# Sthiber/COSC_4397_Pathtracing_Raytracing_Project

Measured on AMD Instinct MI355X. Metric: Msamples/s, cornell.txt 1920x1080 depth 8 (+PSNR vs 5000spp ref), higher is better.
Workload: dtype f32

## Files before the change

### cosc_4397_pathtracing_raytracing_project_amd/capi.py

```python
from __future__ import annotations

import ctypes as C
import os
from typing import Optional, Sequence, Tuple

import numpy as np

_PKG = os.path.dirname(os.path.abspath(__file__))
LIB_PATH = os.environ.get("PT_AMD_LIB") or os.path.join(_PKG, "libpt_amd.so")
PT_MAX_DEPTH = 64
ARITH = {"exact": 0, "fma": 1, "fast": 2}
ARITH_NAMES = {v: k for k, v in ARITH.items()}
FEATURE_PLANES = 3
NOISE_PLANES = 2
NOISE_PIXELS_PER_PARTIAL = 1024
CONVERGENCE_WAVES = 16
CONVERGENCE_CAPACITY = 65536
FLT_MAX = float(np.finfo(np.float32).max)


class PtGeom(C.Structure):
    _fields_ = [("type", C.c_int32), ("materialid", C.c_int32), ("transform", C.c_float * 16),
                ("inverseTransform", C.c_float * 16), ("invTranspose", C.c_float * 16)]

# ... 13 lines not shown
class PtBVHNode(C.Structure):
    _fields_ = [("bmin", C.c_float * 3), ("bmax", C.c_float * 3), ("left", C.c_int32), ("right", C.c_int32),
                ("geomIndex", C.c_int32)]


class PtGridInfo(C.Structure):
    _fields_ = [("res", C.c_int32 * 3), ("origin", C.c_float * 3), ("cell_size", C.c_float * 3), ("pad", C.c_float),
                ("num_cells", C.c_int32), ("num_records", C.c_int32), ("num_leaves", C.c_int32)]


class PtGridRecord(C.Structure):
    _fields_ = [("bmin", C.c_float * 3), ("bmax", C.c_float * 3), ("leaf", C.c_int32), ("neighbours", C.c_int32)]


class PtSceneDesc(C.Structure):
    _fields_ = [("geoms", C.POINTER(PtGeom)), ("num_geoms", C.c_int32), ("materials", C.POINTER(PtMaterial)),
                ("num_materials", C.c_int32), ("camera", PtCamera), ("trace_depth", C.c_int32)]


class PtOptions(C.Structure):
    _fields_ = [("device", C.c_int32), ("pixel_begin", C.c_int32), ("pixel_count", C.c_int32),
                ("iters_per_batch", C.c_int32), ("num_queues", C.c_int32), ("blocks_per_cu", C.c_int32),
                ("time_kernels", C.c_int32), ("legacy_traversal", C.c_int32), ("debug_flags", C.c_int32), ("unfused_primary", C.c_int32), ("unfused_bounces", C.c_int32), ("stripe_pixels", C.c_int32), ("stripe_stride", C.c_int32),
                ("arith", C.c_int32), ("aa_jitter", C.c_int32), ("convergence", C.c_int32),
                ("lds_table_kb", C.c_int32), ("primary_pieces", C.c_int32), ("paths_pieces", C.c_int32), ("paths_min_piece", C.c_int32)]


class PtStats(C.Structure):
    _fields_ = [("samples", C.c_int64), ("live_rays", C.c_int64 * PT_MAX_DEPTH), ("intersect_launches", C.c_int64),
                ("intersect_ms", C.c_double), ("render_ms", C.c_double), ("num_cus", C.c_int32),
                ("grid_blocks", C.c_int32), ("num_queues", C.c_int32), ("iters_per_batch", C.c_int32),
                ("device_bytes", C.c_int64), ("primary_fused", C.c_int32), ("bounces_fused", C.c_int32),
                ("arith", C.c_int32), ("grid_cells", C.c_int32), ("tight_leaves", C.c_int32), ("paths_waves", C.c_int32), ("record_form", C.c_int32),
                ("gather_form", C.c_int32)]


class PtDenoiseOptions(C.Structure):
    _fields_ = [("levels", C.c_int32), ("sigma_color", C.c_float), ("sigma_normal", C.c_float), ("sigma_position", C.c_float),
                ("keep_albedo", C.c_int32)]


class PtSetupTimes(C.Structure):
    _fields_ = [("tables_ms", C.c_double), ("upload_ms", C.c_double), ("buffers_ms", C.c_double), ("probe_ms", C.c_double),
                ("set_camera_ms", C.c_double), ("set_camera_calls", C.c_int32)]


class PtError(RuntimeError):
    pass


_lib: Optional[C.CDLL] = None
_fp = C.POINTER(C.c_float)
_ip = C.POINTER(C.c_int32)


def lib() -> C.CDLL:
    global _lib
    if _lib is not None:
        return _lib
    if not os.path.exists(LIB_PATH):
        raise PtError(f"{LIB_PATH} not found: run `python -c 'import __graft_entry__ as g; g.build()'` "
                      "(hipcc --offload-arch=gfx950).  There is no CPU fallback.")
    L = C.CDLL(LIB_PATH)
    L.pt_last_error.restype = C.c_char_p
    L.pt_scene_load.argtypes = [C.c_char_p, C.c_int, C.c_int, C.POINTER(C.c_void_p)]
    L.pt_scene_free.argtypes = [C.c_void_p]
    L.pt_scene_free.restype = None
# ... 948 lines not shown
```

### cosc_4397_pathtracing_raytracing_project_amd/csrc/pt_api.cpp

```cpp
#include <chrono>
#include <cmath>
#include <cstdarg>
#include <cstdio>
#include <cstring>
#include <string>

#include "pt_adaptive.h"
#include "pt_context.h"
#include "pt_lds.h"
#include "pt_scene.h"
#include "pt_sched.h"

namespace {

std::string g_err;
constexpr int kDebugFlags = 16 | 32 | 64 | 128 | 256 | 512 | ptk::kRetireEveryIteration | 2048 | ptk::kWholeRecords | ptk::kNoFirstBounce | ptk::kRecordsByVisit | ptk::kTileGather;
static_assert(sizeof(PtOptions) == 80, "capi.PtOptions mirrors this layout");
static_assert(PT_CONVERGENCE_WAVES == ptk::kConvWaves, "pt_amd.h documents the size of the convergence metric's partial sums");
}
int pt_fail(const char* fmt, ...) {
  char buf[1024];
  va_list ap;
  va_start(ap, fmt);
  vsnprintf(buf, sizeof(buf), fmt, ap);
  va_end(ap);
  g_err = buf;
  return -1;
}

namespace ptc {
static PtContext* g_default = nullptr;
PtContext* default_context() { return g_default; }

int get_events(Ctx& g, EventPair* ev) {
  if (!g.free_events.empty()) {
    *ev = g.free_events.back();
    g.free_events.pop_back();
    return 0;
  }
  HIP_OK(hipEventCreate(&ev->a));
  HIP_OK(hipEventCreate(&ev->b));
  return 0;
}
static int resolve_events(Ctx& g) {
  auto drain = [&](std::vector<EventPair>& pending, double& total_ms) -> int {
    for (auto& e : pending) {
      float ms = 0;
      HIP_OK(hipEventElapsedTime(&ms, e.a, e.b));
      total_ms += ms;
// ... 50 lines not shown
ptk::BatchInfo tile_batch(const Ctx& g, int iter_first, int K) {
  ptk::BatchInfo b{};
  b.iter_first = iter_first;
  b.K = K;
  b.N = g.N;
  b.pixel_begin = g.pixel_begin;
  b.trace_depth = g.depth;
  b.aa_jitter = g.aa_jitter ? 1 : 0;
  b.stripe = g.stripe;
  b.gap = g.stripe ? g.stripe_stride - g.stripe : 0;
  b.inv_stripe = g.stripe ? 1.0f / (float)g.stripe : 0.0f;
  return b;
}

int run_batch(Ctx& g, int iter_first, int kb) {
  ptk::BatchInfo b = tile_batch(g, iter_first, kb);
  b.slot_shift = g.slot_shift;
  b.flat = g.fuse_bounces ? 0 : 1;
  b.primary_share = primary_share_of(g);
  b.primary_pieces = g.primary_pieces ? g.primary_pieces
                     : ptk::primary_shares(b) ? ptk::auto_shared_pieces(kb, g.qs.nq, g.ret.wq0) : ptk::auto_primary_pieces(kb, g.qs.nq, g.ret.wq0);
  b.paths_pieces = g.paths_pieces;
  const ptk::SceneTables sc = tables(g);
  b.retire_once = ptk::retires_once(b, g.debug_flags) ? 1 : 0;
  b.split_records = ptk::record_form(b, g.debug_flags, ptk::search_form(sc), sc.num_mats);
  if (b.split_records == ptk::kFirstBounce) b.primary_pieces = 1;
  g.record_form = b.split_records;
  b.fixed_slots = ptk::fixed_slots(b, g.debug_flags, ptk::search_form(sc), sc.num_mats, g.ret.seg_cap) ? 1 : 0;
  b.list = g.list;
  if (b.list) b.stripe = 1, b.gap = 0, b.inv_stripe = 1.0f;
  const ptk::KernelApi& k = *g.k;
  auto cnt_row = [&](int d) { return g.d_cnt + ptk::cnt_index(g.qs, d, 0); };
  int d0 = 0;
  if (g.fuse_primary) {
    k.primary(g.stream, g.grid_primary, sc, g.dcam, b, queues_for(g, g.grid_primary), cnt_row(0), cnt_row(1), g.buf[1],
              g.ret);
    d0 = 1;
  } else {
    k.generate(g.stream, g.grid_gen, g.dcam, b, queues_for(g, g.grid_gen), g.buf[0], cnt_row(0));
  }
  int src = d0 & 1;
  const bool all_depths = g.grid_paths > 0;
  EventPair ev{};
  auto timed_from = [&]() -> int {
    if (!g.time_kernels) return 0;
    if (get_events(g, &ev)) return -1;
    HIP_OK(hipEventRecord(ev.a, g.stream));
    return 0;
  };
  auto timed_to = [&]() -> int {
    if (!g.time_kernels) return 0;
    HIP_OK(hipEventRecord(ev.b, g.stream));
    g.pending_isect.push_back(ev);
    return 0;
  };
  if (all_depths) {
    if (timed_from()) return -1;
    k.paths(g.stream, g.grid_paths, sc, b, queues_for(g, g.grid_paths), g.d_cnt, g.buf[1], g.ret);
    if (timed_to()) return -1;
  }
  for (int d = d0; d < g.depth && !all_depths; ++d) {
    const int32_t* cin = cnt_row(d);
    int32_t* cout = cnt_row(d + 1);
    if (timed_from()) return -1;
    k.intersect(g.stream, g.grid_isect, sc, queues_for(g, g.grid_isect), cin, g.buf[src], g.hits, g.legacy, d == 0);
    if (timed_to()) return -1;
    k.shade(g.stream, g.grid_shade, sc, b, d, queues_for(g, g.grid_shade), cin, cout, g.buf[src], g.hits, g.buf[src ^ 1], g.ret);
    src ^= 1;
  }
  ptk::ConvInfo cv{g.d_ref, g.d_partial, -1, kb};
  if (g.conv_live) {
    if (g.conv_have_ref) cv.first_k = 0;
    else if (g.conv >= iter_first && g.conv < iter_first + kb) cv.capture_k = g.conv - iter_first, cv.first_k = cv.capture_k + 1, g.conv_have_ref = true;
    g.conv_last = std::max(g.conv_last, iter_first + kb - 1);
  }
  const bool conv_batch = cv.capture_k >= 0 || cv.first_k < kb;
  g.gather_form = ptk::gather_form(b.fixed_slots != 0, g.debug_flags, conv_batch);
  if (g.gather_form == ptk::kGatherStream) k.collect_stream(g.stream, b, g.qs, g.ret, g.d_image, g.d_cnt, g.depth, g.d_stats);
  else {
    k.count_stats(g.stream, g.qs, g.d_cnt, g.depth, g.d_stats);
    if (conv_batch) k.collect_conv(g.stream, b, g.qs, g.ret, g.d_image, cv, g.d_sse);
    else k.collect(g.stream, b, g.qs, g.ret, g.d_image);
  }
  HIP_OK(hipGetLastError());
  g.samples += (int64_t)kb * g.N;
  if (g.pending_isect.size() > 16384) {
    HIP_OK(hipStreamSynchronize(g.stream));
    if (resolve_events(g)) return -1;
  }
  return 0;
}

void plan_launch(Ctx& g) {
  if (!g.borrowed) g.lds_table_bytes = g.k->lds_table_limit(tables(g), g.lds_table_forced);
  const ptk::SceneTables t = tables(g);
  g.grid_gen = g.num_cus * std::min(g.cap_bpc, g.k->resident_blocks_per_cu(ptk::kGenerate, t));
  g.grid_isect = g.num_cus * std::min(g.cap_bpc, g.k->resident_blocks_per_cu(g.legacy ? ptk::kIntersectLegacy : ptk::kIntersect, t));
  g.grid_shade = g.num_cus * std::min(g.cap_bpc, g.k->resident_blocks_per_cu(ptk::kShade, t));
  g.grid_primary = g.num_cus * std::min(g.cap_bpc, g.k->resident_blocks_per_cu(shares_first_hit(g) ? ptk::kPrimaryShared : ptk::kPrimary, t));
  g.ret.wq0 = ptk::wave_slot(0, g.qs.Q, g.grid_primary * ptk::kWavesPerBlock).wq;
  g.grid_paths = (g.fuse_bounces && g.depth > 1) ? g.num_cus * std::min(g.cap_bpc, g.k->resident_blocks_per_cu(ptk::kPaths, t)) : 0;
  g.qs.paths_W = g.grid_paths * ptk::kWavesPerBlock;
}

static void free_grid(Ctx& g, const Ctx::DeviceGrid& d) {
  for (void* p : {(void*)d.d_start, (void*)d.d_items, d.d_items_b != d.d_items ? (void*)d.d_items_b : nullptr}) {
    if (!p) continue;
    (void)hipFree(p);
    g.allocs.erase(std::remove(g.allocs.begin(), g.allocs.end(), p), g.allocs.end());
  }
  g.device_bytes -= (int64_t)d.bytes;
}
static int choose_traversal(Ctx& g) {
  auto drop_unused_grids = [&](size_t keep) {
    for (size_t i = 0; i < g.grids.size(); ++i)
      if (i != keep) free_grid(g, g.grids[i]);
    g.grids = {g.grids[keep]};
    g.grid_pick = 0;
  };
  if (g.grids.empty()) return 0;
  if (!g.fuse_bounces || (g.debug_flags & (256 | 512))) {
    drop_unused_grids(0);
    return 0;
  }
  auto time_one = [&](float* ms) -> int {
    plan_launch(g);
    for (int rep = 0; rep < 2; ++rep) {
      EventPair ev{};
      if (get_events(g, &ev)) return -1;
      HIP_OK(hipEventRecord(ev.a, g.stream));
      if (run_batch(g, 1, std::min(g.K, 8))) return -1;
      HIP_OK(hipEventRecord(ev.b, g.stream));
      HIP_OK(hipStreamSynchronize(g.stream));
      HIP_OK(hipEventElapsedTime(ms, ev.a, ev.b));
      g.free_events.push_back(ev);
    }
    return 0;
  };
  g.grid_enabled = false;
  if (time_one(&g.probe_ms[0])) return -1;
  g.grid_enabled = true;
  size_t best = 0;
  for (size_t i = 0; i < g.grids.size(); ++i) {
    float ms = 0.f;
    g.grid_pick = i;
    if (time_one(&ms)) return -1;
    if (i == 0 || ms < 0.97f * g.probe_ms[1]) g.probe_ms[1] = ms, best = i;
  }
  drop_unused_grids(best);
  g.grid_enabled = g.probe_ms[1] < 0.95f * g.probe_ms[0];
  plan_launch(g);
  HIP_OK(hipMemsetAsync(g.d_image, 0, 3 * (size_t)g.N * sizeof(float), g.stream));
  HIP_OK(hipMemsetAsync(g.d_stats, 0, PT_MAX_DEPTH * sizeof(unsigned long long), g.stream));
  HIP_OK(hipStreamSynchronize(g.stream));
  g.samples = 0;
  return 0;
}

ptd::Queues single_queue(const Ctx& g, int n) {
  ptd::Queues qs{};
  qs.Q = 1;
  const ptk::QueuePlan p = ptk::queue_plan(n, 1, 1);
  qs.cap = p.cap;
  qs.W = g.grid * ptk::kWavesPerBlock;
  qs.cnt_stride = 16;
  qs.nq = p.nq;
  qs.inv_nq = 1.0f / (float)qs.nq;
  return qs;
}

void destroy(Ctx* c) {
  if (!c) return;
  destroy(c->worker);
  (void)hipSetDevice(c->device);
  if (c->stream) (void)hipStreamSynchronize(c->stream);
  for (void* p : c->allocs) (void)hipFree(p);
  auto kill = [](std::vector<EventPair>& v) {
    for (auto& e : v) {
      (void)hipEventDestroy(e.a);
      (void)hipEventDestroy(e.b);
    }
    v.clear();
  };
  kill(c->free_events);
  kill(c->pending_isect);
  kill(c->pending_render);
  if (c->stream && !c->borrowed) (void)hipStreamDestroy(c->stream);
  delete c;
// ... 121 lines not shown
static int upload_tables(Ctx& g, const pt::HostTables& t) {
  ptk::SceneTables& s = g.scene;
  s.num_nodes = (int)t.nodes.size(), s.num_geoms = (int)t.geoms.size(), s.num_mats = (int)t.mats.size(), s.num_top = (int)t.top.size();
  std::memcpy(s.root_min, t.root_min, 12);
  std::memcpy(s.root_max, t.root_max, 12);
  s.cull_margin = t.cull_margin;
  s.top_xor = t.top_xor;
  s.has_triangles = t.has_triangles ? 1 : 0;
  g.tight_leaves = t.tight_leaves;
  if (!(s.nodes = upload(g, t.nodes)) || !(s.geoms = upload(g, t.geoms)) || !(s.mats = upload(g, t.mats)) || !(s.top = upload(g, t.top))) return -1;
  s.nodes_b = s.nodes, s.top_b = s.top;
  if (!t.nodes_b.empty() && (!(s.nodes_b = upload(g, t.nodes_b)) || !(s.top_b = upload(g, t.top_b)))) return -1;
  for (const pt::Grid& gr : t.grids)
    if (upload_grid(g, gr)) return -1;
  return 0;
}

static __global__ void k_poison_records(ptd::Word4* rec, unsigned long long per_queue, unsigned long long total, int Q) {
  const float nan = __builtin_nanf("");
  for (unsigned long long i = (unsigned long long)blockIdx.x * blockDim.x + threadIdx.x; i < total; i += (unsigned long long)gridDim.x * blockDim.x)
    rec[i] = ptd::Word4{nan, nan, nan, __int_as_float(ptk::chunk_pixel((int)(i / per_queue), 0, Q))};
}

static int poison_records(Ctx& g) {
  const size_t regions = (size_t)g.qs.Q * g.ret.kmax, per_queue = (size_t)g.ret.kmax * g.ret.seg_cap;
  hipLaunchKernelGGL(k_poison_records, dim3((unsigned)std::min<size_t>((regions * g.ret.seg_cap + 255) / 256, 65536)), dim3(256), 0, g.stream, g.ret.rec,
                     (unsigned long long)per_queue, (unsigned long long)(regions * g.ret.seg_cap), g.qs.Q);
  HIP_OK(hipGetLastError());
  return 0;
}
static size_t sub_words_max(const Ctx& g) { return ptk::sub_stride(g.num_cus * 8 * ptk::kWavesPerBlock, g.qs.Q); }

static int rearm_batch_buffers(Ctx& g) {
  for (const ptd::PathBuf& pb : g.buf) HIP_OK(hipMemsetAsync(pb.r, 0xff, pathbuf_words(pb.stride) * sizeof(ptd::Word4), g.stream));
  const size_t regions = (size_t)g.qs.Q * g.ret.kmax;
  HIP_OK(hipMemsetAsync(g.ret.cnt, 0, regions * sizeof(*g.ret.cnt), g.stream));
  HIP_OK(hipMemsetAsync(g.ret.sub, 0, regions * sub_words_max(g) * sizeof(*g.ret.sub), g.stream));
  if (g.qs.deal) HIP_OK(hipMemsetAsync(g.qs.deal, 0, (size_t)ptk::deal_map(g.qs).words() * sizeof(int32_t), g.stream));
  return poison_records(g);
}

int alloc_batch_buffers(Ctx& g) {
  const int Q = g.qs.Q;
  if (alloc_pathbuf(g, &g.buf[0], g.stride) || alloc_pathbuf(g, &g.buf[1], g.stride)) return -1;
  for (const ptd::PathBuf& pb : g.buf) HIP_OK(hipMemset(pb.r, 0xff, pathbuf_words(pb.stride) * sizeof(ptd::Word4)));
  if (!g.fuse_bounces && alloc_hitbuf(g, &g.hits, g.stride)) return -1;
  {
    const size_t regions = (size_t)Q * g.ret.kmax;
    const size_t wq_max = sub_words_max(g);
    if (dalloc(g, &g.ret.rec, regions * g.ret.seg_cap)) return -1;
    if (ensure(g, g.ret.cnt, regions * sizeof(*g.ret.cnt), Zero::blocking) || ensure(g, g.ret.sub, regions * wq_max * sizeof(*g.ret.sub), Zero::blocking)) return -1;
    if (poison_records(g)) return -1;
  }
  const size_t image_bytes = 3 * (size_t)g.N * sizeof(float);
  const size_t cnt_words = ptk::cnt_index(g.qs, g.depth + 1, 0);
  if (ensure(g, g.d_image, image_bytes, Zero::blocking) || ensure(g, g.d_cnt, cnt_words * sizeof(int32_t), Zero::blocking) ||
      ensure(g, g.d_stats, PT_MAX_DEPTH * sizeof(*g.d_stats), Zero::blocking))
    return -1;
  if (!(g.debug_flags & 64) && ensure(g, g.qs.deal, (size_t)ptk::deal_map(g.qs).words() * sizeof(int32_t), Zero::blocking)) return -1;
  if (g.conv) {
    const size_t partials = (size_t)g.K * Q * ptk::kConvWaves;
    if (ensure(g, g.d_ref, image_bytes, Zero::blocking) || ensure(g, g.d_partial, partials * sizeof(double), Zero::blocking)) return -1;
    if (dalloc(g, &g.d_sse, (size_t)PT_CONVERGENCE_CAPACITY)) return -1;
    HIP_OK(hipMemset(g.d_sse, 0xff, (size_t)PT_CONVERGENCE_CAPACITY * sizeof(double)));
  }
  HIP_OK(hipDeviceSynchronize());
// ... 282 lines not shown
  (void)hipFree(d);
  if (e != hipSuccess) return pt_fail("pt_preview_rgba8: %s", hipGetErrorString(e));
  return 0;
}

int pt_ctx_get_stats(PtContext* c, PtStats* out) {
  if (need(c, "pt_get_stats")) return -1;
  if (!out) return pt_fail("pt_get_stats: null");
  if (pt_ctx_sync(c)) return -1;
  Ctx& g = *c;
  std::memset(out, 0, sizeof(*out));
  unsigned long long st[PT_MAX_DEPTH];
  HIP_OK(hipMemcpy(st, g.d_stats, sizeof(st), hipMemcpyDeviceToHost));
  for (int d = 0; d < PT_MAX_DEPTH; ++d) out->live_rays[d] = (int64_t)st[d];
  out->samples = g.samples;
  out->intersect_launches = g.isect_launches;
  out->intersect_ms = g.isect_ms;
  out->render_ms = g.render_ms;
  out->num_cus = g.num_cus;
  out->grid_blocks = g.grid_paths > 0 ? g.grid_paths : g.grid_isect;
  out->num_queues = g.qs.Q;
  out->iters_per_batch = g.K;
  out->device_bytes = g.device_bytes;
  out->primary_fused = g.fuse_primary ? 1 : 0;
  out->bounces_fused = g.fuse_bounces ? 1 : 0;
  out->arith = g.arith;
  if (tables(g).use_grid && g.fuse_bounces) {
    const int* res = g.grids[g.grid_pick].shape.res;
    out->grid_cells = res[0] * res[1] * res[2];
  }
  out->tight_leaves = g.tight_leaves;
  out->record_form = g.record_form;
  out->gather_form = g.gather_form;
  out->paths_waves = 0;
  if (g.qs.deal && g.grid_paths > 0) {
    const ptk::DealMap dm = ptk::deal_map(g.qs);
    std::vector<int32_t> first((size_t)dm.made_for() + 1);
    HIP_OK(hipMemcpy(first.data(), g.qs.deal + dm.first(0), first.size() * sizeof(int32_t), hipMemcpyDeviceToHost));
    if (first[dm.made_for()] == g.qs.paths_W) {
      int lo = first[1] - first[0], hi = lo;
      for (int q = 1; q < g.qs.Q; ++q) lo = std::min(lo, first[q + 1] - first[q]), hi = std::max(hi, first[q + 1] - first[q]);
      out->paths_waves = std::min(lo, 0xffff) << 16 | std::min(hi, 0xffff);
    }
  }
  return 0;
}

int pt_ctx_reset_stats(PtContext* c) {
  if (need(c, "pt_reset_stats")) return -1;
  if (pt_ctx_sync(c)) return -1;
  Ctx& g = *c;
  HIP_OK(hipMemsetAsync(g.d_stats, 0, PT_MAX_DEPTH * sizeof(unsigned long long), g.stream));
  HIP_OK(hipStreamSynchronize(g.stream));
  g.samples = 0;
  g.isect_ms = g.render_ms = 0;
  g.isect_launches = 0;
  return 0;
}

int pt_ctx_clear(PtContext* c) {
  if (need(c, "pt_clear")) return -1;
  if (pt_ctx_sync(c)) return -1;
  HIP_OK(hipMemsetAsync(c->d_image, 0, 3 * (size_t)c->N * sizeof(float), c->stream));
  if (c->d_feat) HIP_OK(hipMemsetAsync(c->d_feat, 0, (size_t)PT_FEATURE_PLANES * c->N * sizeof(float4), c->stream));
  if (c->d_noise) HIP_OK(hipMemsetAsync(c->d_noise, 0, pt_noise_state_bytes((size_t)c->N), c->stream));
  c->noise_groups = 0;
// ... 197 lines not shown
```

### cosc_4397_pathtracing_raytracing_project_amd/csrc/pt_context.h

```cpp
#pragma once
#include <hip/hip_runtime.h>

#include <algorithm>
#include <cstdint>
#include <vector>

#include "../../include/pt_amd.h"
#include "pt_device.h"
#include "pt_internal.h"
#include "pt_kernels.h"
#include "pt_tables.h"

#define HIP_OK(expr)                                                                                      \
  do {                                                                                                    \
    hipError_t e_ = (expr);                                                                               \
    if (e_ != hipSuccess) return pt_fail("%s failed: %s (%s:%d)", #expr, hipGetErrorString(e_), __FILE__, __LINE__); \
  } while (0)

struct EventPair {
  hipEvent_t a, b;
};

struct PtShared {
  int device = 0;
// ... 41 lines not shown
  int grid_gen = 0, grid_isect = 0, grid_shade = 0;
  ptd::Queues qs{};
  int64_t stride = 0;
  std::vector<void*> allocs;
  int64_t device_bytes = 0;
  float probe_ms[2] = {0.f, 0.f};
  int grid_primary = 0, grid_paths = 0;
  ptd::PathBuf buf[2]{};
  ptd::HitBuf hits{};
  ptd::RetireBuf ret{};
  float* d_image = nullptr;
  float4* d_feat = nullptr;
  int grid_features = 0;
  void* d_denoise = nullptr;
  void* d_noise = nullptr;
  int noise_groups = 0;
  int64_t noise_iters = 0;
  int64_t rendered = 0;
  int conv = 0;
  bool conv_live = false;
  bool conv_have_ref = false;
  int conv_last = 0;
  float* d_ref = nullptr;
  double* d_partial = nullptr;
  double* d_sse = nullptr;
  uint8_t* d_rgb8 = nullptr;
  int32_t* d_cnt = nullptr;
  unsigned long long* d_stats = nullptr;
  bool time_kernels = false;
  std::vector<EventPair> free_events, pending_isect, pending_render;
  double isect_ms = 0, render_ms = 0;
  int64_t isect_launches = 0;
  int64_t samples = 0;
  bool failed = false;
  int opt_iters_per_batch = 0, opt_num_queues = 0;
  bool borrowed = false;
  const int32_t* list = nullptr;
  PtContext* worker = nullptr;
  int capacity = 0;
  int32_t* d_list = nullptr;
  int32_t* d_list_frame = nullptr;
  void* d_acnt = nullptr;
  void* d_select = nullptr;
  float* d_resolved = nullptr;
  pt::CameraBase camera_base;
  pt::GridRequest grid_request;
  PtSetupTimes setup_times{};
  bool adaptive = false;
  int adaptive_rounds = 0;
  int64_t adaptive_last = 0;
};

struct PtCtxState {
  bool adaptive;
  int groups;
  int64_t iters;
  int64_t unfolded;
};
PtCtxState pt_ctx_state(const PtContext* c);
int pt_ctx_admit_state(const PtContext* c, const char* who, bool uniform);
int pt_ctx_adaptive_refusal(const PtContext* c, const char* who, int iter_first, int group_iters, float max_fraction, bool folds);
int pt_ctx_camera_refusal(const PtContext* c, const PtCamera* cam, const char* who);
int pt_ctx_enter_adaptive(PtContext* c);

namespace ptc {
using Ctx = PtContext;
// ... 72 lines not shown
```

### cosc_4397_pathtracing_raytracing_project_amd/csrc/pt_kernels.hip

```cpp
#include "pt_kernels.h"

#include <float.h>

#include <type_traits>

#include "pt_lds.h"
#include "pt_sched.h"
#include "pt_portable_math.h"

#ifndef PT_ARITH
#define PT_ARITH 0
#endif
#if PT_ARITH == 0
#define PT_NS arith_exact
#define PT_API_FN api_exact
#elif PT_ARITH == 1
#define PT_NS arith_fma
#define PT_API_FN api_fma
#elif PT_ARITH == 2
#define PT_NS arith_fast
#define PT_API_FN api_fast
#else
#error "PT_ARITH must be 0, 1 or 2"
#endif
// ... 1028 lines not shown
      if (dead) rt.rec[sub0 + nd + rank_in(deadm)] = ptd::Word4{s.c.x, s.c.y, s.c.z, __int_as_float(pl)};
      nl += (int)__popcll(live), nd += (int)__popcll(deadm);
    };
    if constexpr (RING) ws = carry_init<true, 2>(wbase), ws.qo_tab = cam_qo, ws.cam_o = o;
    if constexpr (SHARE && SPLIT == kFirstBounce) {
      const int sub_off = sub_offset(quo, rem, shared_rho(r, 0, wq)) * 64;
      int fnl = 0, fnd = 0;
      auto record_group = [&](unsigned long long best, const float* rec, const Group& g) {
        const bool valid = g.valid;
        const Hit h = resolve_hit(best, rec, valid, leaf_geom);
        const bool cdead = valid && (h.t < 0.0f || mats[h.mat].emittance > 0.0f), lives = valid && !cdead;
        const unsigned long long livem = ballot(lives), cdeadm = ballot(cdead);
        if (lives) path_store(out, qbase + sub_off + fnl + rank_in(livem), bounce_origin(h.n, h.p), h.n, g.d, PathTag{pack_first(g.pl, h.mat, b.slot_shift), g.phash, 0});
        if (cdead) {
          ShadeIO s;
          s.o = o;
          s.d = g.d;
          s.c = mk(1.0f, 1.0f, 1.0f);
          s.alive = false;
          shade_decide(mats, b.trace_depth, 0, iter_hash_of(ihash, sc, b, 0, 0) ^ g.phash, h.t, h.mat, s);
          rt.rec[sub_off + fnd + rank_in(cdeadm)] = ptd::Word4{s.c.x, s.c.y, s.c.z, __int_as_float(g.pl)};
        }
        fnl += (int)__popcll(livem), fnd += (int)__popcll(cdeadm);
      };
      pp.any = false;
      int it = 0;
      for (int jj = shared_rho(r, 0, wq); jj < sh.my_nq; jj += wq, ++it) trace(it, group_of(jj, 0), record_group);
      if constexpr (RING) {
        if (pp.any) {
          carry_drain_to<true, 2, kD0, true>(ws, pp.mark, lane, nodes, geoms);
          record_group(ws.best[pp.par * 64 + lane], ws.rec + pp.par * 6 * 64 + lane, pp.g);
        }
      }
      for (int k = lane; k < b.K; k += 64) rt.sub[k * rt.wq0 + shared_rho(r, k, wq)] = ((unsigned long long)(uint32_t)fnd << 32) | (uint32_t)fnl;
    } else if constexpr (SHARE) {
      const int cap = shared_run_cap(b.primary_share), sub_off = sub_offset(quo, rem, shared_rho(r, k0, wq)) * 64;
      const bool once = b.retire_once != 0;
      for (int run = 0, runs = shared_runs(k0, k1, cap); run < runs; ++run) {
        const Run sr = shared_run(k0, k1, cap, run);
        const int s0 = sr.k0, s1 = sr.k1;
        int vnl = 0, vnd = 0;
        auto shade_run = [&](unsigned long long best, const float* rec, const Group& g) {
          const bool valid = g.valid;
          const int pl = g.pl;
          const uint32_t phash = g.phash;
          const f3 d = g.d;
          const Hit h = resolve_hit(best, rec, valid, leaf_geom);
          const float ht = h.t;
          const int hmat = h.mat;
          const f3 hn = h.n, hp = h.p;
          if constexpr (SPLIT == kSplitRecords) {
            if (s0 == 0) {
              const bool lives = valid && !(ht < 0.0f || mats[hmat].emittance > 0.0f);
              const unsigned long long livem = ballot(lives);
              const f3 o1 = bounce_origin(hn, hp);
              if (lives) out.r[out.stride + qbase + sub_off + __builtin_amdgcn_readlane(vnl, 0) + rank_in(livem)] = ptd::Word4{o1.x, o1.y, o1.z, __int_as_float(hmat)};
            }
          }
          const bool cdead = once && valid && (ht < 0.0f || mats[hmat].emittance > 0.0f);
          const unsigned long long cdeadm = once ? ballot(cdead) : 0ull;
          if (once) {
            if (s0 == 0 && cdeadm) {
              ShadeIO s;
              s.o = o;
              s.d = d;
              s.c = mk(1.0f, 1.0f, 1.0f);
              s.alive = false;
// ... 237 lines not shown
    tword[e] = (uint32_t)leaf | ((uint32_t)gi << 8);
    lmat[leaf & 63] = sc.geoms[gi].material;
  }
  __syncthreads();
  const int wib = threadIdx.x >> 6;
  char* wbase = lds + L.waves + wib * L.wave_bytes;
  Lanes cy = lanes_init(wbase);
  GridRings gr = grid_rings_init<false>(wbase);
  Carry<false, 1>& cb = gr.cy;
  CellRing& cr = gr.cr;
  cb.lnodes = (const __attribute__((address_space(3))) v4f*)(lnodes ? lnodes : lds), cb.lds_nodes = lnodes != nullptr;
  constexpr bool SLOTS = MODE == 0;
  char* slots = wbase + WM::slots;
  int* died = reinterpret_cast<int*>(wbase + WM::died);
  [[maybe_unused]] int* fillc = reinterpret_cast<int*>(wbase + WM::fillc);
  const int ntop = sc.num_top;
  const int wave = __builtin_amdgcn_readfirstlane(blockIdx.x * kWavesPerBlock + wib);
  const int lane = lane_id();
  died[lane] = 0;
  const uint64_t t_begin = __builtin_amdgcn_s_memrealtime();
  const DealMap dm = deal_map(qs);
  const WaveSlot even = wave_slot(wave, qs.Q, qs.W);
  int q = even.q, r = even.r, wq = even.wq;
  if (qs.deal != nullptr && qs.deal[dm.made_for()] == qs.W) {
    int at_or_before = 0;
    for (int e0 = 0; e0 < qs.Q; e0 += 64) at_or_before += (int)__popcll(ballot(e0 + lane < qs.Q && qs.deal[dm.first(e0 + lane)] <= wave));
    q = at_or_before - 1;
    const int first = qs.deal[dm.first(q)];
    r = wave - first, wq = qs.deal[dm.first(q + 1)] - first;
  }
  const Retire rt = retire_of(ret, q);
  const int64_t qbase = (int64_t)q * qs.cap;
  const int wq0 = rt.wq0, ne = b.K * wq0;
  const int my_nq = queue_share(b, qs, q).my_nq, quo = my_nq / wq0, rem = my_nq % wq0;
  auto count_of = [&](int e) { return e < ne ? (int)(uint32_t)rt.sub[e] : 0; };
  int total = 0, csum = 0;
  const bool chunk_sums = ne <= 64 * 64;
  for (int e0 = 0; e0 < ne; e0 += 256) {
    int n4[4];
#pragma unroll
    for (int j = 0; j < 4; ++j) n4[j] = count_of(e0 + 64 * j + lane);
#pragma unroll
    for (int j = 0; j < 4; ++j) {
      int sum;
      (void)wave_prefix6(n4[j], sum);
      total += sum;
      if (lane == (e0 >> 6) + j) csum = sum;
    }
  }
  if (r == 0 && lane == 0) cnt[cnt_index(qs, 1, q)] = total;
  const PiecePlan pieces = piece_plan(total, wq, b.paths_pieces, qs.deal != nullptr, chunk_sums);
  [[maybe_unused]] int clist0 = 0;
  int ce = ne, cstart = total, ccnt = 0, clist = 0;
  int cord = 0;
  [[maybe_unused]] int cur_k = 0;
  [[maybe_unused]] uint32_t cur_h = 0u, next_h = 0u;
  [[maybe_unused]] int crec0 = 0;
  [[maybe_unused]] const int fbits = fixed_bits(rt.seg_cap);
  int win0 = -64;
  unsigned long long wsub = 0ull;
  auto window_to = [&](int e) {
    if (e < win0 || e >= win0 + 64) {
      win0 = e;
      wsub = (e + lane < ne) ? rt.sub[e + lane] : 0ull;
    }
  };
  auto sub_word = [&](int e) -> unsigned long long {
    const uint32_t lo32 = (uint32_t)__builtin_amdgcn_readlane((int)(uint32_t)wsub, e - win0);
    const uint32_t hi32 = (uint32_t)__builtin_amdgcn_readlane((int)(uint32_t)(wsub >> 32), e - win0);
    return ((unsigned long long)hi32 << 32) | lo32;
  };
  window_to(0);
  auto cursor_bases = [&](int first_rank) {
    const int ec = min(ce, ne - 1), ck = ec / wq0, crho = ec - ck * wq0;
    clist = ck * rt.seg_cap + sub_offset(quo, rem, crho) * 64;
    if constexpr (SPLIT != 0) clist0 = invariant_slot(clist, ck, rt.seg_cap);
    if constexpr (FIRST) cur_k = ck, cur_h = iter_hash(b.iter_first + ck, 0);
    window_to(ec);
    const int crec = clist + (int)(uint32_t)(sub_word(ec) >> 32);
    if constexpr (FIXED) crec0 = invariant_slot(crec, ck, rt.seg_cap);
    else if (lane == 0) fillc[cord & (kVisitRing - 1)] = crec + (first_rank - cstart);
  };
  auto seek = [&](int at_rank) {
// ... 395 lines not shown
```

### cosc_4397_pathtracing_raytracing_project_amd/csrc/pt_post.cpp

```cpp
#include <cmath>

#include "pt_adaptive.h"
#include "pt_context.h"
#include "pt_denoise.h"
#include "pt_noise.h"
#include "pt_sched.h"

using namespace ptc;

int64_t pt_ctx_unfolded_iterations(const PtContext* c) { return c ? c->rendered - c->noise_iters : 0; }

extern "C" {

int pt_ctx_render_features(PtContext* c, int iter_first, int iter_count) {
  if (need(c, "pt_render_features")) return -1;
  Ctx& g = *c;
  if (iter_first < 1 || iter_count < 0 || (int64_t)iter_first + iter_count - 1 > INT32_MAX)
    return pt_fail("pt_render_features: iterations %d, +%d: the first is >= 1, the count >= 0", iter_first, iter_count);
  if (admit(g, "pt_render_features", kNotFailed | kOnDevice)) return -1;
  const ptk::SceneTables sc = tables(g);
  static_assert(sizeof(float4) == 16, "a feature plane holds 16 bytes per pixel");
  if (ensure(g, g.d_feat, (size_t)PT_FEATURE_PLANES * g.N * sizeof(float4), Zero::on_stream)) return -1;
  if (iter_count == 0) return 0;
  const int groups = (g.N + 63) / 64;
// ... 141 lines not shown
void set_worker_live(Ctx& w, int m) {
  const ptk::QueuePlan plan = ptk::queue_plan(m, w.qs.Q, w.K);
  w.N = m;
  w.qs.nq = plan.nq;
  w.qs.inv_nq = 1.0f / (float)plan.nq;
  w.qs.cap = plan.cap;
  w.stride = (int64_t)w.qs.Q * plan.cap;
  w.ret.seg_cap = plan.seg_cap;
}

int ensure_worker(Ctx& g, int m) {
  if (g.worker && g.worker->capacity == m) return set_worker_live(*g.worker, m), 0;
  if (g.worker) g.device_bytes -= g.worker->device_bytes, destroy(g.worker), g.worker = nullptr;
  if (ensure(g, g.d_list, (size_t)g.N * sizeof(int32_t), Zero::blocking)) return -1;
  if (g.stripe && ensure(g, g.d_list_frame, (size_t)g.N * sizeof(int32_t), Zero::blocking)) return -1;
  Ctx* w = new Ctx();
  w->borrowed = true;
  static_cast<PtShared&>(*w) = g;
  PtOptions o{};
  o.pixel_begin = g.pixel_begin, o.pixel_count = m;
  o.iters_per_batch = g.opt_iters_per_batch, o.num_queues = g.opt_num_queues;
  if (plan_batches(*w, o)) return destroy(w), -1;
  plan_launch(*w);
  if (alloc_batch_buffers(*w)) return destroy(w), -1;
  w->list = g.stripe ? g.d_list_frame : g.d_list;
  w->capacity = m;
  g.worker = w;
  g.device_bytes += w->device_bytes;
  return 0;
}

int render_list(Ctx& g, int iter_first, int iter_count) {
  Ctx& w = *g.worker;
  HIP_OK(hipMemsetAsync(w.d_image, 0, 3 * (size_t)w.N * sizeof(float), g.stream));
  const int end = iter_first + iter_count;
  for (int it = iter_first; it < end; it += w.K)
    if (run_batch(w, it, std::min(w.K, end - it))) {
      g.failed = true;
      return -1;
    }
  return 0;
}

static int adaptive_refusal(const Ctx& g, const char* who, int iter_first, int group_iters, const float* fraction_or_null, bool folds = true,
                            bool rows = true) {
  const float fraction = fraction_or_null ? *fraction_or_null : 1.0f;
  if (admit(g, who, kNotFailed)) return -1;
  if (folds && (iter_first < 1 || group_iters < 1 || (int64_t)iter_first + group_iters - 1 > INT32_MAX))
    return pt_fail("%s: iterations %d, +%d: the first is >= 1, the group holds at least one", who, iter_first, group_iters);
  if (!folds && iter_first < 1) return pt_fail("%s: the first iteration %d is not >= 1", who, iter_first);
  if (!(fraction > 0.0f && fraction <= 1.0f)) return pt_fail("%s: fraction %g is not in (0, 1]", who, (double)fraction);
  if (g.conv) return pt_fail("%s: the renderer was created with PtOptions.convergence = %d; the convergence metric follows whole iterations", who, g.conv);
  if (rows && admit(g, who, kWholeRows)) return -1;
  if (g.adaptive || !folds) return 0;
  if (g.noise_groups < 2) return pt_fail("%s: %d group(s) folded; the selection needs the noise estimate of at least 2 (pt_noise_fold)", who, g.noise_groups);
  if (admit(g, who, kFoldedAll)) return -1;
  if (g.noise_iters > INT32_MAX / 2) return pt_fail("%s: %lld iterations folded: the per-pixel counts are int32", who, (long long)g.noise_iters);
  return 0;
}

static int enter_adaptive(Ctx& g) {
  if (g.adaptive) return 0;
  if (ensure(g, g.d_acnt, (size_t)g.N * sizeof(ptad::Cnt))) return -1;
  if (pt_adaptive_init_counts_launch(g.stream, g.N, g.d_acnt, (int)g.noise_iters, g.noise_groups)) return -1;
  g.adaptive = true;
  g.adaptive_rounds = 0;
// ... 210 lines not shown
```

### cosc_4397_pathtracing_raytracing_project_amd/csrc/pt_sched.h

```cpp
#pragma once
#include "pt_kernels.h"

#define PT_SCHED __host__ __device__ inline __attribute__((always_inline))

namespace ptk {

PT_SCHED int sched_min(int a, int b) { return a < b ? a : b; }
PT_SCHED int sched_max(int a, int b) { return a > b ? a : b; }

struct DealMap {
  int Q;
  PT_SCHED int first(int q) const { return q; }
  PT_SCHED int made_for() const { return Q; }
  PT_SCHED int time(int q) const { return Q + 1 + q; }
  PT_SCHED int strand_counter() const { return 2 * Q + 1; }
  PT_SCHED int piece_counter(int q) const { return 2 * Q + 2 + q; }
  PT_SCHED int rays(int q) const { return 3 * Q + 2 + q; }
  PT_SCHED int words() const { return 4 * Q + 2; }
};
PT_SCHED DealMap deal_map(const ptd::Queues& qs) { return DealMap{qs.Q}; }

PT_SCHED int dealt_first(int q, int W, int Q, unsigned long long work_before, unsigned long long work_total) {
  return q + (int)((unsigned long long)(W - Q) * work_before / work_total);
}
// ... 120 lines not shown
PT_SCHED bool splits_records(const BatchInfo& b, int debug_flags) {
  return splits_records(b.primary_share, b.aa_jitter != 0, b.flat != 0, b.trace_depth, debug_flags);
}
PT_SCHED int invariant_slot(int at, int k, int seg_cap) { return at - k * seg_cap; }
PT_SCHED uint32_t pack_kind(int sample_id, bool specular) { return (uint32_t)sample_id | (specular ? 0x80000000u : 0u); }
PT_SCHED int kind_sample_id(uint32_t word) { return (int)(word & 0x7fffffffu); }
PT_SCHED bool kind_specular(uint32_t word) { return (word >> 31) != 0u; }

constexpr int kNoFirstBounce = 8192;
constexpr int kSplitRecords = 1, kFirstBounce = 2;
constexpr int kVisitBits = 8;
PT_SCHED uint32_t pack_visit(int k, int visit) { return ((uint32_t)k << kVisitBits) | ((uint32_t)visit & ((1u << kVisitBits) - 1u)); }
PT_SCHED int visit_k(uint32_t word) { return (int)(word >> kVisitBits); }
PT_SCHED int visit_number(uint32_t word) { return (int)(word & ((1u << kVisitBits) - 1u)); }
PT_SCHED int visit_gap(int visits_now, int visit) { return (visits_now - visit) & ((1 << kVisitBits) - 1); }
PT_SCHED bool visit_k_fits(int K) { return K <= (1 << (31 - kVisitBits)); }
PT_SCHED int pack_first(int pl, int mat, int slot_shift) { return (mat << slot_shift) | pl; }
PT_SCHED int first_pixel(int word, int slot_shift) { return word & ((1 << slot_shift) - 1); }
PT_SCHED int first_material(int word, int slot_shift) { return (int)((uint32_t)word >> slot_shift); }
PT_SCHED bool first_material_fits(int num_mats, int slot_shift) { return num_mats <= (1 << (31 - slot_shift)); }
PT_SCHED bool first_bounces(int primary_share, bool aa_jitter, bool flat, int trace_depth, int debug_flags, int search_form, int num_mats,
                            int slot_shift, int K) {
  return splits_records(primary_share, aa_jitter, flat, trace_depth, debug_flags) &&
         retires_once(primary_share, aa_jitter, flat, trace_depth, debug_flags) && !(debug_flags & kNoFirstBounce) && search_form == 0 &&
         first_material_fits(num_mats, slot_shift) && visit_k_fits(K);
}
PT_SCHED bool first_bounces(const BatchInfo& b, int debug_flags, int search_form, int num_mats) {
  return first_bounces(b.primary_share, b.aa_jitter != 0, b.flat != 0, b.trace_depth, debug_flags, search_form, num_mats, b.slot_shift, b.K);
}
PT_SCHED int record_form(const BatchInfo& b, int debug_flags, int search_form, int num_mats) {
  return first_bounces(b, debug_flags, search_form, num_mats) ? kFirstBounce : splits_records(b, debug_flags) ? kSplitRecords : 0;
}

constexpr int kRecordsByVisit = 16384, kTileGather = 32768;
constexpr int kFixedSlots = 3;
PT_SCHED int fixed_slot(int k, int seg_cap, int quo, int rem, int rho, int retirees, int i) { return k * seg_cap + sub_offset(quo, rem, rho) * 64 + retirees + i; }
PT_SCHED int fixed_bits(int seg_cap) { return 32 - __builtin_clz((unsigned)(seg_cap - 1)); }
PT_SCHED uint32_t pack_fixed(int k, int in_region, int bits) { return ((uint32_t)k << bits) | (uint32_t)in_region; }
PT_SCHED int fixed_k(uint32_t word, int bits) { return (int)(word >> bits); }
PT_SCHED int fixed_slot_of(uint32_t word, int bits, int seg_cap) { return (int)(word >> bits) * seg_cap + (int)(word & ((1u << bits) - 1u)); }
PT_SCHED bool fixed_word_fits(int K, int seg_cap) { return K <= (1 << (31 - fixed_bits(seg_cap))); }
PT_SCHED bool fixed_slots(int primary_share, bool aa_jitter, bool flat, int trace_depth, int debug_flags, int search_form, int num_mats, int slot_shift,
                          int K, int seg_cap) {
  return first_bounces(primary_share, aa_jitter, flat, trace_depth, debug_flags, search_form, num_mats, slot_shift, K) && fixed_word_fits(K, seg_cap) &&
         !(debug_flags & kRecordsByVisit);
}
PT_SCHED bool fixed_slots(const BatchInfo& b, int debug_flags, int search_form, int num_mats, int seg_cap) {
  return fixed_slots(b.primary_share, b.aa_jitter != 0, b.flat != 0, b.trace_depth, debug_flags, search_form, num_mats, b.slot_shift, b.K, seg_cap);
}
constexpr int kGatherTile = 0, kGatherTileFixed = 1, kGatherStream = 2;
PT_SCHED int gather_form(bool fixed, int debug_flags, bool convergence) { return !fixed ? kGatherTile : (debug_flags & kTileGather) || convergence ? kGatherTileFixed : kGatherStream; }

PT_SCHED int pack_paths_pieces(int count, int min_piece) { return count | min_piece << 16; }
PT_SCHED int paths_pieces_count(int word) { return word & 0xffff; }
PT_SCHED int paths_pieces_min(int word) { return word >> 16; }
struct PieceRange {
  int start, end;
  bool some;
};
struct PiecePlan {
  int total, wq, pieces_per_wave, ps_min, ps0;
  PT_SCHED bool needs_counter() const { return ps0 * wq < total; }
  PT_SCHED PieceRange piece_range(int nextp) const {
    int start = total, sz = ps0;
    if (nextp >= 0) {
      start = 0;
      int level = nextp / wq;
      const int idx = nextp - level * wq;
      for (; level > 0 && start < total; --level) start += wq * sz, sz = sched_max(sz - sz / pieces_per_wave, ps_min);
      start += idx * sz;
    }
    return start < total ? PieceRange{start, sched_min(start + sz, total), true} : PieceRange{total, total, false};
  }
};
PT_SCHED PiecePlan piece_plan(int total, int wq, int paths_pieces, bool deal_present, bool chunk_sums) {
  PiecePlan p;
  p.total = total, p.wq = wq;
  p.pieces_per_wave = deal_present && chunk_sums && paths_pieces_count(paths_pieces) > 1 ? paths_pieces_count(paths_pieces) : 1;
  p.ps_min = paths_pieces_min(paths_pieces);
  p.ps0 = sched_max((total + wq * p.pieces_per_wave - 1) / (wq * p.pieces_per_wave), p.ps_min);
  return p;
// ... 4 lines not shown
```

### include/pt_amd.h

```cpp
#ifndef PT_AMD_H
#define PT_AMD_H

#include <stdint.h>

#ifdef __cplusplus
extern "C" {
#endif

#define PT_GEOM_SPHERE 0
#define PT_GEOM_CUBE 1
#define PT_GEOM_TRIANGLE 2

typedef struct PtGeom {
  int32_t type;
  int32_t materialid;
  float transform[16];
  float inverseTransform[16];
  float invTranspose[16];
} PtGeom;

typedef struct PtMaterial {
  float color[3];
  float specular_exponent;
  float specular_color[3];
// ... 44 lines not shown
  int32_t stripe_pixels;
  int32_t stripe_stride;
  int32_t arith;
  int32_t aa_jitter;
  int32_t convergence;
  int32_t lds_table_kb;
  int32_t primary_pieces;
  int32_t paths_pieces;
  int32_t paths_min_piece;
} PtOptions;
#define PT_PRIMARY_PIECES(pieces, share) ((int32_t)((pieces) | (share) << 16))

#define PT_ARITH_EXACT 0
#define PT_ARITH_FMA 1
#define PT_ARITH_FAST 2

#define PT_MAX_DEPTH 64
typedef struct PtStats {
  int64_t samples;
  int64_t live_rays[PT_MAX_DEPTH];
  int64_t intersect_launches;
  double intersect_ms;
  double render_ms;
  int32_t num_cus, grid_blocks, num_queues, iters_per_batch;
  int64_t device_bytes;
  int32_t primary_fused;
  int32_t bounces_fused;
  int32_t arith;
  int32_t grid_cells;
  int32_t tight_leaves;
  int32_t paths_waves;
  int32_t record_form;
  int32_t gather_form;
} PtStats;

typedef struct PtScene PtScene;
int pt_scene_load(const char* path, int res_w, int res_h, PtScene** out);
void pt_scene_free(PtScene* s);
int pt_scene_desc(const PtScene* s, PtSceneDesc* out);
int pt_scene_iterations(const PtScene* s);
int pt_scene_orbit(PtScene* s, float dphi, float dtheta, float dzoom);
int pt_scene_camera(const PtScene* s, PtCamera* out);
int pt_scene_orbit_state(const PtScene* s, float* phi, float* theta, float* zoom);
const char* pt_scene_image_name(const PtScene* s);

int pt_build_bvh(const PtGeom* geoms, int num_geoms, PtBVHNode* out, int cap);

typedef struct PtGridInfo {
  int32_t res[3];
  float origin[3], cell_size[3], pad;
  int32_t num_cells, num_records, num_leaves;
} PtGridInfo;
typedef struct PtGridRecord {
  float bmin[3], bmax[3];
  int32_t leaf;
  int32_t neighbours;
} PtGridRecord;
int pt_build_grid(const PtGeom* geoms, int num_geoms, int forced, PtGridInfo* info, uint32_t* cell_start, PtGridRecord* records);

int pt_traversal_boxes(const PtGeom* geoms, int num_geoms, const float camera_position[3], float* boxes);

void pt_center_half_box(const float lo[3], const float hi[3], int inner, float magnitude, float center[3], float half_extent[3]);

int pt_build_transform(const float* trs, float* transform, float* inverse, float* invTranspose);

int pt_init(const PtSceneDesc* scene, const PtOptions* opt);
// ... 203 lines not shown
```

Baseline: 40130.

## Reuse fused primary-ray results across batches when slots are fixed and deterministic

When primary rays are deterministic (no AA jitter) and the fixed-slot record form applies, the fused primary kernel is now skipped on later batches. A key made of scene tables, camera, batch layout, queues and buffers is compared against the previous launch. The primary kernel now writes the first-bounce records for all kmax slots, and the paths kernel fills in the depth-0 count itself, so the cached records stay valid. This removes a repeated full-screen primary trace per batch, but it depends on the retire buffers not being overwritten between batches, and it adds invalidation points that must cover every state change.

```diff
diff --git a/cosc_4397_pathtracing_raytracing_project_amd/capi.py b/cosc_4397_pathtracing_raytracing_project_amd/capi.py
--- a/cosc_4397_pathtracing_raytracing_project_amd/capi.py
+++ b/cosc_4397_pathtracing_raytracing_project_amd/capi.py
@@ -69,7 +69,7 @@
                 ("grid_blocks", C.c_int32), ("num_queues", C.c_int32), ("iters_per_batch", C.c_int32),
                 ("device_bytes", C.c_int64), ("primary_fused", C.c_int32), ("bounces_fused", C.c_int32),
                 ("arith", C.c_int32), ("grid_cells", C.c_int32), ("tight_leaves", C.c_int32), ("paths_waves", C.c_int32), ("record_form", C.c_int32),
-                ("gather_form", C.c_int32)]
+                ("gather_form", C.c_int32), ("primary_launches", C.c_int64)]
 
 
 class PtDenoiseOptions(C.Structure):
diff --git a/cosc_4397_pathtracing_raytracing_project_amd/csrc/pt_api.cpp b/cosc_4397_pathtracing_raytracing_project_amd/csrc/pt_api.cpp
--- a/cosc_4397_pathtracing_raytracing_project_amd/csrc/pt_api.cpp
+++ b/cosc_4397_pathtracing_raytracing_project_amd/csrc/pt_api.cpp
@@ -14,7 +14,7 @@
 namespace {
 
 std::string g_err;
-constexpr int kDebugFlags = 16 | 32 | 64 | 128 | 256 | 512 | ptk::kRetireEveryIteration | 2048 | ptk::kWholeRecords | ptk::kNoFirstBounce | ptk::kRecordsByVisit | ptk::kTileGather;
+constexpr int kDebugFlags = 16 | 32 | 64 | 128 | 256 | 512 | ptk::kRetireEveryIteration | 2048 | ptk::kWholeRecords | ptk::kNoFirstBounce | ptk::kRecordsByVisit | ptk::kTileGather | ptk::kPrimaryEveryBatch;
 static_assert(sizeof(PtOptions) == 80, "capi.PtOptions mirrors this layout");
 static_assert(PT_CONVERGENCE_WAVES == ptk::kConvWaves, "pt_amd.h documents the size of the convergence metric's partial sums");
 }
@@ -131,9 +131,20 @@
   const ptk::KernelApi& k = *g.k;
   auto cnt_row = [&](int d) { return g.d_cnt + ptk::cnt_index(g.qs, d, 0); };
   int d0 = 0;
+  const bool once = g.fuse_primary && ptk::primary_once(b, g.debug_flags, ptk::search_form(sc), sc.num_mats, g.ret.seg_cap);
+  const bool had_first_hits = g.primary_valid;
+  g.primary_valid = false;
   if (g.fuse_primary) {
-    k.primary(g.stream, g.grid_primary, sc, g.dcam, b, queues_for(g, g.grid_primary), cnt_row(0), cnt_row(1), g.buf[1],
-              g.ret);
+    const ptd::Queues pq = queues_for(g, g.grid_primary);
+    Ctx::PrimaryKey key;
+    std::memset(&key, 0, sizeof(key));
+    key.sc = sc, key.cam = g.dcam, key.b = b, key.b.iter_first = key.b.K = 0, key.qs = pq, key.out = g.buf[1], key.ret = g.ret;
+    key.kernels = &k, key.grid = g.grid_primary, key.debug_flags = g.debug_flags;
+    if (!(once && had_first_hits && std::memcmp(&key, &g.primary_key, sizeof(key)) == 0)) {
+      k.primary(g.stream, g.grid_primary, sc, g.dcam, b, pq, cnt_row(0), cnt_row(1), g.buf[1], g.ret);
+      g.primary_launches += 1;
+      std::memcpy(&g.primary_key, &key, sizeof(key));
+    }
     d0 = 1;
   } else {
     k.generate(g.stream, g.grid_gen, g.dcam, b, queues_for(g, g.grid_gen), g.buf[0], cnt_row(0));
@@ -182,6 +193,7 @@
     else k.collect(g.stream, b, g.qs, g.ret, g.d_image);
   }
   HIP_OK(hipGetLastError());
+  g.primary_valid = once;
   g.samples += (int64_t)kb * g.N;
   if (g.pending_isect.size() > 16384) {
     HIP_OK(hipStreamSynchronize(g.stream));
@@ -200,6 +212,7 @@
   g.ret.wq0 = ptk::wave_slot(0, g.qs.Q, g.grid_primary * ptk::kWavesPerBlock).wq;
   g.grid_paths = (g.fuse_bounces && g.depth > 1) ? g.num_cus * std::min(g.cap_bpc, g.k->resident_blocks_per_cu(ptk::kPaths, t)) : 0;
   g.qs.paths_W = g.grid_paths * ptk::kWavesPerBlock;
+  g.primary_valid = false;
 }
 
 static void free_grid(Ctx& g, const Ctx::DeviceGrid& d) {
@@ -253,6 +266,7 @@
   HIP_OK(hipMemsetAsync(g.d_stats, 0, PT_MAX_DEPTH * sizeof(unsigned long long), g.stream));
   HIP_OK(hipStreamSynchronize(g.stream));
   g.samples = 0;
+  g.primary_launches = 0;
   return 0;
 }
 
@@ -440,6 +454,7 @@
 static size_t sub_words_max(const Ctx& g) { return ptk::sub_stride(g.num_cus * 8 * ptk::kWavesPerBlock, g.qs.Q); }
 
 static int rearm_batch_buffers(Ctx& g) {
+  g.primary_valid = false;
   for (const ptd::PathBuf& pb : g.buf) HIP_OK(hipMemsetAsync(pb.r, 0xff, pathbuf_words(pb.stride) * sizeof(ptd::Word4), g.stream));
   const size_t regions = (size_t)g.qs.Q * g.ret.kmax;
   HIP_OK(hipMemsetAsync(g.ret.cnt, 0, regions * sizeof(*g.ret.cnt), g.stream));
@@ -788,6 +803,7 @@
   out->tight_leaves = g.tight_leaves;
   out->record_form = g.record_form;
   out->gather_form = g.gather_form;
+  out->primary_launches = g.primary_launches;
   out->paths_waves = 0;
   if (g.qs.deal && g.grid_paths > 0) {
     const ptk::DealMap dm = ptk::deal_map(g.qs);
diff --git a/cosc_4397_pathtracing_raytracing_project_amd/csrc/pt_context.h b/cosc_4397_pathtracing_raytracing_project_amd/csrc/pt_context.h
--- a/cosc_4397_pathtracing_raytracing_project_amd/csrc/pt_context.h
+++ b/cosc_4397_pathtracing_raytracing_project_amd/csrc/pt_context.h
@@ -97,6 +97,19 @@
   double isect_ms = 0, render_ms = 0;
   int64_t isect_launches = 0;
   int64_t samples = 0;
+  struct PrimaryKey {
+    ptk::SceneTables sc;
+    ptd::Camera cam;
+    ptk::BatchInfo b;
+    ptd::Queues qs;
+    ptd::PathBuf out;
+    ptd::RetireBuf ret;
+    const void* kernels;
+    int32_t grid, debug_flags;
+  };
+  PrimaryKey primary_key{};
+  bool primary_valid = false;
+  int64_t primary_launches = 0;
   bool failed = false;
   int opt_iters_per_batch = 0, opt_num_queues = 0;
   bool borrowed = false;
diff --git a/cosc_4397_pathtracing_raytracing_project_amd/csrc/pt_kernels.hip b/cosc_4397_pathtracing_raytracing_project_amd/csrc/pt_kernels.hip
--- a/cosc_4397_pathtracing_raytracing_project_amd/csrc/pt_kernels.hip
+++ b/cosc_4397_pathtracing_raytracing_project_amd/csrc/pt_kernels.hip
@@ -1084,7 +1084,7 @@
           record_group(ws.best[pp.par * 64 + lane], ws.rec + pp.par * 6 * 64 + lane, pp.g);
         }
       }
-      for (int k = lane; k < b.K; k += 64) rt.sub[k * rt.wq0 + shared_rho(r, k, wq)] = ((unsigned long long)(uint32_t)fnd << 32) | (uint32_t)fnl;
+      for (int k = lane; k < ret.kmax; k += 64) rt.sub[k * rt.wq0 + shared_rho(r, k, wq)] = ((unsigned long long)(uint32_t)fnd << 32) | (uint32_t)fnl;
     } else if constexpr (SHARE) {
       const int cap = shared_run_cap(b.primary_share), sub_off = sub_offset(quo, rem, shared_rho(r, k0, wq)) * 64;
       const bool once = b.retire_once != 0;
@@ -1388,7 +1388,8 @@
   const Retire rt = retire_of(ret, q);
   const int64_t qbase = (int64_t)q * qs.cap;
   const int wq0 = rt.wq0, ne = b.K * wq0;
-  const int my_nq = queue_share(b, qs, q).my_nq, quo = my_nq / wq0, rem = my_nq % wq0;
+  const QueueShare qshare = queue_share(b, qs, q);
+  const int my_nq = qshare.my_nq, quo = my_nq / wq0, rem = my_nq % wq0;
   auto count_of = [&](int e) { return e < ne ? (int)(uint32_t)rt.sub[e] : 0; };
   int total = 0, csum = 0;
   const bool chunk_sums = ne <= 64 * 64;
@@ -1405,6 +1406,8 @@
     }
   }
   if (r == 0 && lane == 0) cnt[cnt_index(qs, 1, q)] = total;
+  if constexpr (SPLIT == kFirstBounce || SPLIT == kFixedSlots)
+    if (r == 0 && lane == 0) cnt[cnt_index(qs, 0, q)] = b.K * qshare.my_pixels;
   const PiecePlan pieces = piece_plan(total, wq, b.paths_pieces, qs.deal != nullptr, chunk_sums);
   [[maybe_unused]] int clist0 = 0;
   int ce = ne, cstart = total, ccnt = 0, clist = 0;
diff --git a/cosc_4397_pathtracing_raytracing_project_amd/csrc/pt_post.cpp b/cosc_4397_pathtracing_raytracing_project_amd/csrc/pt_post.cpp
--- a/cosc_4397_pathtracing_raytracing_project_amd/csrc/pt_post.cpp
+++ b/cosc_4397_pathtracing_raytracing_project_amd/csrc/pt_post.cpp
@@ -197,6 +197,7 @@
 
 int render_list(Ctx& g, int iter_first, int iter_count) {
   Ctx& w = *g.worker;
+  w.primary_valid = false;
   HIP_OK(hipMemsetAsync(w.d_image, 0, 3 * (size_t)w.N * sizeof(float), g.stream));
   const int end = iter_first + iter_count;
   for (int it = iter_first; it < end; it += w.K)
diff --git a/cosc_4397_pathtracing_raytracing_project_amd/csrc/pt_sched.h b/cosc_4397_pathtracing_raytracing_project_amd/csrc/pt_sched.h
--- a/cosc_4397_pathtracing_raytracing_project_amd/csrc/pt_sched.h
+++ b/cosc_4397_pathtracing_raytracing_project_amd/csrc/pt_sched.h
@@ -176,6 +176,8 @@
   return first_bounces(b, debug_flags, search_form, num_mats) ? kFirstBounce : splits_records(b, debug_flags) ? kSplitRecords : 0;
 }
 
+constexpr int kPrimaryEveryBatch = 65536;
+
 constexpr int kRecordsByVisit = 16384, kTileGather = 32768;
 constexpr int kFixedSlots = 3;
 PT_SCHED int fixed_slot(int k, int seg_cap, int quo, int rem, int rho, int retirees, int i) { return k * seg_cap + sub_offset(quo, rem, rho) * 64 + retirees + i; }
@@ -191,6 +193,13 @@
 }
 PT_SCHED bool fixed_slots(const BatchInfo& b, int debug_flags, int search_form, int num_mats, int seg_cap) {
   return fixed_slots(b.primary_share, b.aa_jitter != 0, b.flat != 0, b.trace_depth, debug_flags, search_form, num_mats, b.slot_shift, b.K, seg_cap);
+}
+PT_SCHED bool primary_once(int primary_share, bool aa_jitter, bool flat, int trace_depth, int debug_flags, int search_form, int num_mats, int slot_shift,
+                           int K, int seg_cap) {
+  return fixed_slots(primary_share, aa_jitter, flat, trace_depth, debug_flags, search_form, num_mats, slot_shift, K, seg_cap) && !(debug_flags & kPrimaryEveryBatch);
+}
+PT_SCHED bool primary_once(const BatchInfo& b, int debug_flags, int search_form, int num_mats, int seg_cap) {
+  return primary_once(b.primary_share, b.aa_jitter != 0, b.flat != 0, b.trace_depth, debug_flags, search_form, num_mats, b.slot_shift, b.K, seg_cap);
 }
 constexpr int kGatherTile = 0, kGatherTileFixed = 1, kGatherStream = 2;
 PT_SCHED int gather_form(bool fixed, int debug_flags, bool convergence) { return !fixed ? kGatherTile : (debug_flags & kTileGather) || convergence ? kGatherTileFixed : kGatherStream; }
diff --git a/include/pt_amd.h b/include/pt_amd.h
--- a/include/pt_amd.h
+++ b/include/pt_amd.h
@@ -100,6 +100,7 @@
   int32_t paths_waves;
   int32_t record_form;
   int32_t gather_form;
+  int64_t primary_launches;
 } PtStats;
 
 typedef struct PtScene PtScene;
```

Measured after the change: 41050 (median of 6 runs). 1.02x the previous value.
